# LLSean/ACE-Step-1.5-ggml

Measured on AMD Instinct MI355X. Metric: DiT denoising steps/sec (240s@5Hz latent, bs=1..8) + single-step ms; 1/2/4/8 GPU, higher is better.
Workload: dtype bf16

## Files before the change

ace-step-1.5-ggml_amd/csrc/kernels/gemm.hip:

```cpp
#include <array>
#include <cstdio>
#include <cstdlib>
#include <mutex>
#include <map>
#include <vector>
#include <type_traits>
#include <utility>

#include "gemm_common.h"

namespace acemi {
namespace gemm_detail {

#ifndef ACEMI_GEMM_ABLATE
#define ACEMI_GEMM_ABLATE 0
#endif
constexpr int kAblate = ACEMI_GEMM_ABLATE;


template <int TBM, int TBN, int TWM, int TWN, int TEPI, int TPIPE, bool TSK>
struct GemmTwoPerCU {
    static constexpr bool value =
        (TSK || ((TEPI == EPI_RESID || TEPI == EPI_RESID_GATED) && TPIPE >= 1 && TWM * TWN == 4 &&
                 (TBM / TWM / 16) * 4 * (TBN / TWN / 16) + (TEPI == EPI_RESID_GATED ? 2 * (TBN / TWN / 16) : 0) <= 63)) &&
// ... 193 lines not shown
            if (kt + 1 < nk) {
                if constexpr (PF)
                    wait_vmcnt<XW>();
                else
                    wait_retire(min(kt + NS, nk - 1) - (kt + 1));
                __builtin_amdgcn_s_barrier();
            }
        };
        if constexpr (XPF) {
            const int kp = nk >= 2 ? nk - 2 : 0;
            for (int kt = 0; kt < kp; ++kt) body(kt, std::false_type{});
            body(kp, std::true_type{});
            if (kp + 1 < nk) body(kp + 1, std::false_type{});
            resid_apply<TM, TN, EPI>(p, acc, m0 + wm0, n0 + wn0, lane, BM / WM, xo, g0, g1);
            return;
        } else {
            for (int kt = 0; kt < nk; ++kt) body(kt, std::false_type{});
        }
    }

    if constexpr (SK)
        if (!splitk_join<TM, TN, NW, SplitKMax<BM, BN>::value, NS * STAGE>(p, acc, S, sk_tile, sk_part, tid, smem,
                                                                                ticket0))
            return;
    if constexpr (EPI == EPI_QKV_PREP)
        qkv_prep_tile<BM, NW, TM, TN, NS * STAGE>(p, acc, m0, n0, wm0, wn0, tid, smem);
    else
        gemm_epilogue<TM, TN, F16, EPI, (SK ? 32 : (NW > 4 ? NW : 1024))>(p, acc, m0 + wm0, n0 + wn0, lane);
}


template <int BM, int BN, bool F16, int EPI, int NS>
__global__ void __launch_bounds__(512, 1) gemm_ws_kernel(GemmParams p) {
    constexpr int NC = 4, WN = 2;
    constexpr int WTM = BM / 2, WTN = BN / WN;
    constexpr int TM = WTM / 16, TN = WTN / 16;
    constexpr int BK = 64, ROWB = BK * 2;
    constexpr int STAGE = (BM + BN) * ROWB;
    constexpr int G = (BM + BN) / 8 / 4;
    static_assert((BM + BN) % 32 == 0 && NS >= 3, "ws tile");
    static_assert(EPI != EPI_SWIGLU || (TN % 2 == 0), "swiglu needs column pairs");
    __shared__ __attribute__((aligned(16))) char smem[NS * STAGE];

    const int tid = threadIdx.x, lane = tid & 63, wid = tid >> 6;
    int m0, n0;
    block_tile<BM, BN>(p, m0, n0);
    const int nk = p.K / BK;
    const uint32_t lds0 = (uint32_t)(uintptr_t)(__attribute__((address_space(3))) char*)smem;

    if (wid >= NC) {
        const int lw = wid - NC;
        const uint16_t* src[G];
#pragma unroll
        for (int j = 0; j < G; ++j) {
            const int row = (lw + 4 * j) * 8 + (lane >> 3);
            const int c = (lane & 7) ^ swz(row);
            src[j] = row < BM ? p.A + (int64_t)min(m0 + row, p.M - 1) * p.lda + c * 8
                              : p.W + (int64_t)(n0 + row - BM) * p.ldw + c * 8;
        }
        auto stage = [&](int slot, int kt) {
#pragma unroll
            for (int j = 0; j < G; ++j)
                __builtin_amdgcn_global_load_lds((const void*)(src[j] + kt * BK),
                                                 (lds_void*)(smem + slot * STAGE + (lw + 4 * j) * 1024), 16, 0, 0);
        };
        auto wait_tiles = [&](int n) {
            if (NS >= 4 && n >= 3) wait_vmcnt<(NS >= 4 ? 3 : 0) * G>();
            else if (n == 2) wait_vmcnt<2 * G>();
            else if (n == 1) wait_vmcnt<G>();
            else wait_vmcnt<0>();
        };
#pragma unroll
        for (int t = 0; t < NS; ++t)
            if (t < nk) stage(t, t);
        wait_tiles(min(NS, nk) - 1);
        __builtin_amdgcn_s_barrier();
        for (int j = 1; j < nk; ++j) {
            wait_tiles(min(nk - 1, j - 2 + NS) - j);
            __builtin_amdgcn_s_barrier();
            if (j - 1 + NS < nk) stage((j - 1) % NS, j - 1 + NS);
        }
        wait_vmcnt<0>();
        if constexpr (EPI == EPI_QKV_PREP)
            qkv_prep_head<BM, 8, NS * STAGE>(p, m0, n0 >> 7, tid, smem, [](float*, int, int) {});
        return;
    }

    const int wm0 = (wid / WN) * WTM, wn0 = (wid % WN) * WTN;
    const int lrow = lane & 15, lchunk = lane >> 4;
    const int rsw = (lrow >> 1) & 7;
    const uint32_t ch[2] = {(uint32_t)((lchunk ^ rsw) * 16), (uint32_t)(((4 + lchunk) ^ rsw) * 16)};
    f32x4 acc[TM][TN];
#pragma unroll
    for (int i = 0; i < TM; ++i)
#pragma unroll
        for (int j = 0; j < TN; ++j) acc[i][j] = f32x4{0.f, 0.f, 0.f, 0.f};
    uint4 a[TM][2], b[TN][2];
    auto rd = [&](auto r_c, int slot, auto h_c) {
        constexpr int r = decltype(r_c)::value, h = decltype(h_c)::value;
        const uint32_t sb = lds0 + slot * STAGE + ch[h];
        if constexpr (r < TN)
            b[r][h] = ds_read_b128_off<r * 16 * ROWB>(sb + (BM + wn0 + lrow) * ROWB);
        else
            a[r - TN][h] = ds_read_b128_off<(r - TN) * 16 * ROWB>(sb + (wm0 + lrow) * ROWB);
    };
    auto half = [&](auto h_c, int slot, auto hr_c, auto reads_c) {
        constexpr int h = decltype(h_c)::value;
        static_for<0, TM * TN>([&](auto s_c) {
            constexpr int st = decltype(s_c)::value;
            acc[st / TN][st % TN] = mfma16<F16>(a[st / TN][h], b[st % TN][h], acc[st / TN][st % TN]);
            if constexpr (decltype(reads_c)::value && st < TM + TN) rd(s_c, slot, hr_c);
            __builtin_amdgcn_sched_barrier(0);
        });
    };
    using H0 = std::integral_constant<int, 0>;
    using H1 = std::integral_constant<int, 1>;
    __builtin_amdgcn_s_barrier();
    static_for<0, TM + TN>([&](auto r_c) { rd(r_c, 0, H0{}); });
    lds_wait_all();
    using RD = std::true_type;
    for (int kt = 0; kt < nk - 1; ++kt) {
        half(H0{}, kt % NS, H1{}, RD{});
        lds_wait_all();
        __builtin_amdgcn_s_barrier();
        half(H1{}, (kt + 1) % NS, H0{}, RD{});
        lds_wait_all();
    }
    half(H0{}, (nk - 1) % NS, H1{}, RD{});
    lds_wait_all();
    half(H1{}, 0, H0{}, std::false_type{});
    if constexpr (EPI == EPI_QKV_PREP)
        qkv_prep_head<BM, 8, NS * STAGE>(p, m0, n0 >> 7, tid, smem, [&](float* tile, int c0, int CH) {
            const int ccol = lane & 15, crow = (lane >> 4) * 4;
#pragma unroll
            for (int i = 0; i < TM; ++i) {
                const int rb = wm0 + i * 16 - c0;
                if (rb < 0 || rb >= CH) continue;
#pragma unroll
                for (int r = 0; r < 4; ++r)
#pragma unroll
                    for (int j = 0; j < TN; ++j) tile[(rb + crow + r) * PREP_LD + wn0 + j * 16 + ccol] = acc[i][j][r];
            }
        });
    else
        gemm_epilogue<TM, TN, F16, EPI, 64>(p, acc, m0 + wm0, n0 + wn0, lane);
}

template <int BM, bool F16, int EPI, bool SK = false>
__global__ void __launch_bounds__(512) gemm8_kernel(GemmParams p) {
    constexpr int BN = 256, BK = 64, ROWB = BK * 2;
    constexpr int HA = BM / 2;
    constexpr int QM = BM / 64;
    constexpr int QN = 2;
    constexpr int PA = HA / 8;
    constexpr int STAGE = (BM + BN) * ROWB;
    constexpr int SCRATCH = 2 * STAGE;
    static_assert(BM == 256 || BM == 192, "gemm8 tile rows");
    static_assert(EPI != EPI_SWIGLU || (QN % 2 == 0), "swiglu needs column pairs");

    __shared__ __attribute__((aligned(16))) char smem[2 * STAGE + 16 * 1024];

    const int tid = threadIdx.x;
    const int lane = tid & 63;
    const int wid = tid >> 6;
    const int wr = wid >> 2, wc = wid & 3;
    int m0, n0, sk_tile = 0, sk_part = 0;
    unsigned ticket0 = 0;
    const int S = SK ? p.ksplit : 1;
    if constexpr (SK) {
        int ntiles;
        splitk_block(S, sk_tile, sk_part, ntiles);
        block_tile<BM, BN>(p, m0, n0, sk_tile, ntiles);
        if (tid == 0) ticket0 = __hip_atomic_fetch_add(p.sk_cnt + sk_tile, 1u, __ATOMIC_RELAXED, __HIP_MEMORY_SCOPE_AGENT);
    } else {
        block_tile<BM, BN>(p, m0, n0);
    }
    const int M = p.M;
    const int nk_all = p.K / BK;
    const int kt_begin = sk_part * nk_all / S;
    const int nk = (sk_part + 1) * nk_all / S - kt_begin;

    constexpr bool A2 = PA == 16;
    const bool a_second = A2 || wid + 8 < PA;
    const int prow = wid * 8 + (lane >> 3);
    const int pch = (lane & 7) ^ swz(prow);
    const uint16_t* srcA[2][2];
    const uint16_t* srcB[2][2];
#pragma unroll
    for (int h = 0; h < 2; ++h)
#pragma unroll
        for (int j = 0; j < 2; ++j) {
            const int ra = min(m0 + h * HA + j * 64 + prow, M - 1);
            srcA[h][j] = p.A + (int64_t)ra * p.lda + pch * 8 + kt_begin * BK;
            srcB[h][j] = p.W + (int64_t)(n0 + h * 128 + j * 64 + prow) * p.ldw + pch * 8 + kt_begin * BK;
        }
    auto stage_a = [&](int h, int t) {
        char* dst = t < nk ? smem + (t & 1) * STAGE + h * HA * ROWB : smem + SCRATCH;
        const int kt = min(t, nk - 1);
        __builtin_amdgcn_global_load_lds((const void*)(srcA[h][0] + kt * BK), (lds_void*)(dst + wid * 1024), 16, 0, 0);
        if (a_second)
            __builtin_amdgcn_global_load_lds((const void*)(srcA[h][1] + kt * BK), (lds_void*)(dst + (wid + 8) * 1024),
                                             16, 0, 0);
    };
    auto stage_b = [&](int h, int t) {
        char* dst = t < nk ? smem + (t & 1) * STAGE + (BM + h * 128) * ROWB : smem + SCRATCH;
        const int kt = min(t, nk - 1);
        __builtin_amdgcn_global_load_lds((const void*)(srcB[h][0] + kt * BK), (lds_void*)(dst + wid * 1024), 16, 0, 0);
        __builtin_amdgcn_global_load_lds((const void*)(srcB[h][1] + kt * BK), (lds_void*)(dst + (wid + 8) * 1024), 16,
                                         0, 0);
    };
    auto wait_stages = [&]() {
        if (a_second)
            wait_vmcnt<8>();
        else
            wait_vmcnt<6>();
    };

    const uint32_t lds0 = (uint32_t)(uintptr_t)(__attribute__((address_space(3))) char*)smem;
    const int lrow = lane & 15, lchunk = lane >> 4;
    const int rsw = (lrow >> 1) & 7;
    auto read_a = [&](int buf, int h, uint4 (&a)[QM][2]) {
        const uint32_t base = lds0 + buf * STAGE + (h * HA + wr * QM * 16 + lrow) * ROWB;
#pragma unroll
        for (int kk = 0; kk < 2; ++kk) ReadRows<0, QM, 16 * ROWB>::run(base + (((kk * 4 + lchunk) ^ rsw) * 16), a, kk);
// ... 3 lines not shown
#pragma unroll
        for (int kk = 0; kk < 2; ++kk) ReadRows<0, QN, 16 * ROWB>::run(base + (((kk * 4 + lchunk) ^ rsw) * 16), b, kk);
    };

    f32x4 acc[2][2][QM][QN];
#pragma unroll
    for (int x = 0; x < 2; ++x)
#pragma unroll
        for (int y = 0; y < 2; ++y)
#pragma unroll
            for (int i = 0; i < QM; ++i)
#pragma unroll
                for (int j = 0; j < QN; ++j) acc[x][y][i][j] = f32x4{0.f, 0.f, 0.f, 0.f};

    auto mma = [&](const uint4 (&a)[QM][2], const uint4 (&b)[QN][2], f32x4 (&c)[QM][QN]) {
        __builtin_amdgcn_s_setprio(1);
#pragma unroll
        for (int kk = 0; kk < 2; ++kk)
#pragma unroll
            for (int i = 0; i < QM; ++i)
#pragma unroll
                for (int j = 0; j < QN; ++j) c[i][j] = mfma16<F16>(a[i][kk], b[j][kk], c[i][j]);
        mfma_war_retire(a, b);
        __builtin_amdgcn_s_setprio(0);
    };
    auto seg = [&]() { __builtin_amdgcn_s_barrier(); };

    stage_a(0, 0);
    stage_b(0, 0);
    stage_b(1, 0);
    stage_a(1, 0);
    stage_a(0, 1);
    stage_b(0, 1);
    wait_stages();
    __builtin_amdgcn_s_barrier();
    if (wr == 1) __builtin_amdgcn_s_barrier();

    uint4 a[QM][2], b0[QN][2], b1[QN][2];
    for (int kt = 0; kt < nk; ++kt) {
        const int buf = kt & 1;
        if (!(kAblate & 2) || kt == 0) {
            read_a(buf, 0, a);
            read_b(buf, 0, b0);
        }
        if (!(kAblate & 1)) stage_b(1, kt + 1);
        wait_stages();
        seg();
        lds_wait_all();
        mma(a, b0, acc[0][0]);
        seg();
        if (!(kAblate & 2) || kt == 0) read_b(buf, 1, b1);
        if (!(kAblate & 1)) stage_a(1, kt + 1);
        wait_stages();
        seg();
        lds_wait_all();
        mma(a, b1, acc[0][1]);
        seg();
        if (!(kAblate & 2) || kt == 0) read_a(buf, 1, a);
        if (!(kAblate & 1)) stage_a(0, kt + 2);
        seg();
        lds_wait_all();
        mma(a, b1, acc[1][1]);
        seg();
        if (!(kAblate & 1)) stage_b(0, kt + 2);
        wait_stages();
        seg();
        __builtin_amdgcn_sched_barrier(0);
        mma(a, b0, acc[1][0]);
        seg();
    }
    if (wr == 0) __builtin_amdgcn_s_barrier();
    wait_vmcnt<0>();
    if constexpr (SK) {
        auto& acc2 = reinterpret_cast<f32x4 (&)[4 * QM][QN]>(acc);
        if (!splitk_join<4 * QM, QN, 8, SplitKMax<BM, BN>::value, 2 * STAGE + 16 * 1024>(p, acc2, S, sk_tile, sk_part, tid,
                                                                                        smem, ticket0))
            return;
    }

    if constexpr (EPI == EPI_QKV_PREP) {
        const int ccol = lane & 15, crow = (lane >> 4) * 4;
#pragma unroll
        for (int hb = 0; hb < 2; ++hb)
            qkv_prep_head<BM, 8, 2 * STAGE>(p, m0, (n0 >> 7) + hb, tid, smem, [&](float* tile, int c0, int CH) {
#pragma unroll
                for (int ha = 0; ha < 2; ++ha)
#pragma unroll
                    for (int i = 0; i < QM; ++i) {
                        const int rb = ha * HA + wr * QM * 16 + i * 16 - c0;
                        if (rb < 0 || rb >= CH) continue;
#pragma unroll
                        for (int r = 0; r < 4; ++r)
#pragma unroll
                            for (int j = 0; j < QN; ++j)
                                tile[(rb + crow + r) * PREP_LD + wc * 32 + j * 16 + ccol] = acc[ha][hb][i][j][r];
                    }
            });
    } else {
#pragma unroll
        for (int ha = 0; ha < 2; ++ha)
#pragma unroll
            for (int hb = 0; hb < 2; ++hb)
                gemm_epilogue<QM, QN, F16, EPI, 64>(p, acc[ha][hb], m0 + ha * HA + wr * QM * 16,
                                                   n0 + hb * 128 + wc * 32, lane);
    }
}

struct SplitKWs {
    void* ws = nullptr;
    size_t ws_bytes = 0;
    unsigned* cnt = nullptr;
    size_t tiles = 0;
};
std::mutex g_sk_mu;
std::map<std::pair<int, hipStream_t>, SplitKWs> g_sk;
std::map<int, unsigned*> g_sk_err;

unsigned* splitk_err_word(int dev) {
    unsigned*& e = g_sk_err[dev];
    if (!e) {
        ACEMI_HIP(hipHostMalloc(reinterpret_cast<void**>(&e), sizeof(unsigned), hipHostMallocMapped));
        *reinterpret_cast<volatile unsigned*>(e) = 0u;
    }
    return e;
}

void splitk_setup(GemmParams& p, int ntiles, int S, size_t tile_bytes, hipStream_t s) {
    int dev = 0;
    ACEMI_HIP(hipGetDevice(&dev));
    std::lock_guard<std::mutex> lk(g_sk_mu);
    SplitKWs& w = g_sk[std::make_pair(dev, s)];
    const size_t need = (size_t)ntiles * S * tile_bytes;
    if (w.ws_bytes < need || w.tiles < (size_t)ntiles) ACEMI_HIP(hipStreamSynchronize(s));
    if (w.ws_bytes < need) {
        if (w.ws) ACEMI_HIP(hipFree(w.ws));
        w.ws = nullptr;
        w.ws_bytes = 0;
        ACEMI_HIP(hipMalloc(&w.ws, need));
        w.ws_bytes = need;
    }
    if (w.tiles < (size_t)ntiles) {
        if (w.cnt) ACEMI_HIP(hipFree(w.cnt));
        w.cnt = nullptr;
        w.tiles = 0;
        const size_t t = std::max<size_t>((size_t)ntiles, 4096);
        ACEMI_HIP(hipMalloc(&w.cnt, 2 * t * sizeof(unsigned)));
        ACEMI_HIP(hipMemsetAsync(w.cnt, 0, 2 * t * sizeof(unsigned), s));
        w.tiles = t;
    }
    unsigned* err = splitk_err_word(dev);
    unsigned* err_dev = nullptr;
    ACEMI_HIP(hipHostGetDevicePointer(reinterpret_cast<void**>(&err_dev), err, 0));
    p.ksplit = S;
    p.sk_ws = static_cast<f32x4*>(w.ws);
    p.sk_cnt = w.cnt;
    p.sk_ready = w.cnt + w.tiles;
    p.sk_err = err_dev;
}

template <int BM, int BN, int WM, int WN, bool F16, int EPI, int PIPE, bool SK>
void launch_cfg(GemmParams p, int S, hipStream_t s) {
    static_assert(!SK || (WM * WN == 4 && PIPE >= 1), "split-K is for the 4-wave pipelined tiles");
    const int nbm = (p.M + BM - 1) / BM;
    const int nbn = p.N / BN;
    const dim3 grid(nbm * nbn * (S > 1 ? S : 1));
    const dim3 block(WM * WN * 64);
    if constexpr (EPI == EPI_QKV_PREP && BN != 128) {
        throw std::runtime_error("gemm: the fused attention prep needs 128-wide column tiles");
    } else {
        if constexpr (SK) {
            if (S > 1) {
                if (S > SplitKMax<BM, BN>::value) throw std::runtime_error("gemm: split-K factor too large for this tile");
                splitk_setup(p, nbm * nbn, S, (size_t)BM * BN * 4, s);
                hipLaunchKernelGGL((gemm_kernel<BM, BN, WM, WN, F16, EPI, PIPE, true>), grid, block, 0, s, p);
                return;
            }
        }
        hipLaunchKernelGGL((gemm_kernel<BM, BN, WM, WN, F16, EPI, PIPE>), grid, block, 0, s, p);
// ... 143 lines not shown
```

ace-step-1.5-ggml_amd/csrc/kernels/gemm_common.h:

```cpp
#pragma once

#include <algorithm>
#include <cmath>
#include <cstdlib>
#include <stdexcept>
#include <type_traits>

#include "../gemm_variants.h"
#include "../kernels.h"
#include "prep_math.h"
#include "mfma_guard.h"

namespace acemi {
namespace gemm_detail {

typedef __attribute__((ext_vector_type(8))) __bf16 bf16x8;
typedef __attribute__((ext_vector_type(8))) _Float16 f16x8;
typedef __attribute__((ext_vector_type(4))) float f32x4;

typedef __attribute__((address_space(3))) void lds_void;

struct GemmParams {
    const uint16_t* A;
    const uint16_t* W;
// ... 185 lines not shown
                        if (e.bias) v = v + bias_j[j];
                        e.c_act[(int64_t)m * e.ldc + n] = to_act<F16>(v);
                    } else if constexpr (EPI == EPI_PROJ_OUT) {
                        const int item = m / e.rows_per_item;
                        const int pp = m - item * e.rows_per_item;
                        const int kpos = n / e.out_ch;
                        const int c = n - kpos * e.out_ch;
                        const int t = pp * e.patch + kpos;
                        if (t < e.out_T) {
                            e.c_f32[((int64_t)item * e.out_T + t) * e.out_ch + c] = rn_add(v, e.bias[c]);
                        }
                    }
                }
            }
        }
    }
}

template <int TM, int TN, int EPI>
__device__ __forceinline__ void resid_prefetch(const GemmParams& p, int mw, int nw, int lane, int wrows,
                                               float (&xo)[TM][4][TN], float (&g0)[TN], float (&g1)[TN]) {
    const GemmEpilogue& e = p.e;
    const int ccol = lane & 15, crow = (lane >> 4) * 4;
#pragma unroll
    for (int i = 0; i < TM; ++i)
#pragma unroll
        for (int r = 0; r < 4; ++r) {
            const int m = min(mw + i * 16 + crow + r, p.M - 1);
#pragma unroll
            for (int j = 0; j < TN; ++j) xo[i][r][j] = e.c_f32[(int64_t)m * e.ldc + nw + j * 16 + ccol];
        }
    if constexpr (EPI == EPI_RESID_GATED) {
        const int i0 = min(mw, p.M - 1) / e.rows_per_item, i1 = min(mw + wrows - 1, p.M - 1) / e.rows_per_item;
#pragma unroll
        for (int j = 0; j < TN; ++j) {
            const int n = nw + j * 16 + ccol;
            g0[j] = e.gate[(int64_t)i0 * e.gate_stride + n];
            g1[j] = e.gate[(int64_t)i1 * e.gate_stride + n];
        }
    }
}

template <int TM, int TN, int EPI>
__device__ __forceinline__ void resid_apply(const GemmParams& p, f32x4 (&acc)[TM][TN], int mw, int nw, int lane,
                                            int wrows, const float (&xo)[TM][4][TN], const float (&g0)[TN],
                                            const float (&g1)[TN]) {
    const GemmEpilogue& e = p.e;
    const int ccol = lane & 15, crow = (lane >> 4) * 4;
    const int i0 = min(mw, p.M - 1) / e.rows_per_item;
    if (EPI != EPI_RESID_GATED || e.rows_per_item >= wrows) {
#pragma unroll
        for (int i = 0; i < TM; ++i)
#pragma unroll
            for (int r = 0; r < 4; ++r) {
                const int m = mw + i * 16 + crow + r;
                if (m >= p.M) continue;
                const bool first = m / e.rows_per_item == i0;
#pragma unroll
                for (int j = 0; j < TN; ++j) {
                    float v = acc[i][j][r];
                    if constexpr (EPI == EPI_RESID_GATED) v = rn_mul(v, first ? g0[j] : g1[j]);
                    e.c_f32[(int64_t)m * e.ldc + nw + j * 16 + ccol] = rn_add(xo[i][r][j], v);
                }
            }
    } else {
#pragma unroll
        for (int i = 0; i < TM; ++i)
#pragma unroll
            for (int r = 0; r < 4; ++r) {
                const int m = mw + i * 16 + crow + r;
                if (m >= p.M) continue;
                const int item = m / e.rows_per_item;
#pragma unroll
                for (int j = 0; j < TN; ++j) {
                    const int n = nw + j * 16 + ccol;
                    const float v = rn_mul(acc[i][j][r], e.gate[(int64_t)item * e.gate_stride + n]);
                    e.c_f32[(int64_t)m * e.ldc + n] = rn_add(xo[i][r][j], v);
                }
            }
    }
}

constexpr int PREP_LD = 144;

template <int BM, int NW, int SMEM, class Fill>
__device__ __forceinline__ void qkv_prep_head(const GemmParams& p, int m0, int hd, int tid, char* smem, Fill fill) {
    constexpr int LD = PREP_LD;
    constexpr int CH = (BM * LD * 4 <= SMEM) ? BM : ((BM / 2) * LD * 4 <= SMEM ? BM / 2 : BM / 4);
    static_assert(CH * LD * 4 <= SMEM && BM % CH == 0 && CH % 16 == 0, "qkv prep chunking");
    constexpr int NT = NW * 64;
    const PrepArgs& a = p.e.prep;
    float* tile = reinterpret_cast<float*>(smem);
    const int nq = a.q_col >= 0 ? a.hq : 0;
    const int nk = a.k_col >= 0 ? a.hkv : 0;
    for (int c0 = 0; c0 < BM; c0 += CH) {
        const int mc0 = m0 + c0;
        if (mc0 >= p.M) break;
        __syncthreads();
        fill(tile, c0, CH);
        __syncthreads();
        const int rows = min(CH, p.M - mc0);
        if (hd < nq + nk) {
            const bool isq = hd < nq;
            const int head = isq ? hd : hd - nq;
            const float* w = isq ? a.q_norm : a.k_norm;
            uint16_t* base = isq ? a.qh + (int64_t)head * a.n_pad * 128 : a.kh + (int64_t)head * a.n_pad * 128;
            const int64_t bstride = (int64_t)(isq ? a.hq : a.hkv) * a.n_pad * 128;
            const int64_t plane = isq ? a.q_plane : a.k_plane;
            const int d = (tid & 15) * 4;
            for (int t = tid >> 4; t < rows; t += NT / 16) {
                const int m = mc0 + t;
                const int b = m / a.n_tok, n = m - b * a.n_tok;
                const float4 x0 = *(const float4*)(tile + t * LD + d), x1 = *(const float4*)(tile + t * LD + 64 + d);
                float y[8] = {x0.x, x0.y, x0.z, x0.w, x1.x, x1.y, x1.z, x1.w};
                prep::head_row(y, w, d, a.eps, a.rope_cos ? a.rope_cos + (int64_t)n * 64 + d : nullptr,
                               a.rope_cos ? a.rope_sin + (int64_t)n * 64 + d : nullptr,
                               base + b * bstride + (int64_t)n * 128, plane, a.f8 ? (isq ? 1 : 2) : 0);
            }
        } else {
            const int hk = hd - nq - nk;
            const int d = tid & 127;
            const int b_lo = mc0 / a.n_tok, b_hi = (mc0 + rows - 1) / a.n_tok;
            for (int b = b_lo; b <= b_hi; ++b) {
                const int n_lo = max(0, mc0 - b * a.n_tok), n_hi = min(a.n_tok, mc0 + rows - b * a.n_tok);
                uint16_t* vdst = a.vt + (((int64_t)b * a.hkv + hk) * 128 + d) * a.n_pad;
                const int g_end = n_hi == a.n_tok ? a.n_pad / 16 : ((n_hi - 1) >> 4) + 1;
                for (int g = (n_lo >> 4) + (tid >> 7); g < g_end; g += NT / 128) {
                    const int g0 = g * 16;
                    float v[16];
                    uint32_t have = 0;
#pragma unroll
                    for (int k = 0; k < 16; ++k) {
                        const int n = g0 + prep::vperm(k);
                        const bool mine = n >= n_lo && n < n_hi;
                        v[k] = mine ? tile[(b * a.n_tok + n - mc0) * LD + d] : 0.f;
                        have |= (mine || n >= a.n_tok) ? (1u << k) : 0u;
                    }
                    uint32_t wv[8], wl[8];
                    prep::v_words(v, wv, wl);
                    if (a.f8 && a.v_plane > 0) {
                        float vn[16];
                        uint32_t hn = 0;
#pragma unroll
                        for (int w = 0; w < 16; ++w) {
                            vn[w] = v[prep::vperm(w)];
                            hn |= ((have >> prep::vperm(w)) & 1u) << w;
                        }
                        prep::v_store8(vn, vdst, a.v_plane, g0, hn);
                    }
                    if (have == 0xffffu) {
                        *(uint4*)(vdst + g0) = make_uint4(wv[0], wv[1], wv[2], wv[3]);
                        *(uint4*)(vdst + g0 + 8) = make_uint4(wv[4], wv[5], wv[6], wv[7]);
                        if (a.v_plane > 0 && !a.f8) {
                            *(uint4*)(vdst + a.v_plane + g0) = make_uint4(wl[0], wl[1], wl[2], wl[3]);
                            *(uint4*)(vdst + a.v_plane + g0 + 8) = make_uint4(wl[4], wl[5], wl[6], wl[7]);
                        }
                    } else {
#pragma unroll
                        for (int k = 0; k < 16; ++k) {
                            if (!((have >> k) & 1u)) continue;
                            vdst[g0 + k] = (uint16_t)(wv[k >> 1] >> (16 * (k & 1)));
                            if (a.v_plane > 0 && !a.f8) vdst[a.v_plane + g0 + k] = (uint16_t)(wl[k >> 1] >> (16 * (k & 1)));
                        }
                    }
                }
            }
        }
    }
}

template <int BM, int NW, int TM, int TN, int SMEM>
__device__ __forceinline__ void qkv_prep_tile(const GemmParams& p, f32x4 (&acc)[TM][TN], int m0, int n0, int wm0,
                                              int wn0, int tid, char* smem) {
    const int lane = tid & 63;
    const int ccol = lane & 15, crow = (lane >> 4) * 4;
    qkv_prep_head<BM, NW, SMEM>(p, m0, n0 >> 7, tid, smem, [&](float* tile, int c0, int CH) {
#pragma unroll
        for (int i = 0; i < TM; ++i) {
            const int rb = wm0 + i * 16 - c0;
            if (rb < 0 || rb >= CH) continue;
#pragma unroll
            for (int r = 0; r < 4; ++r)
#pragma unroll
                for (int j = 0; j < TN; ++j) tile[(rb + crow + r) * PREP_LD + wn0 + j * 16 + ccol] = acc[i][j][r];
        }
    });
}

constexpr int CPOL_SC1 = 16;

template <int BM, int BN>
struct SplitKMax {
    static constexpr int value = BM * BN >= 128 * 128 ? 2 : 4;
};

__device__ __forceinline__ void splitk_block(int S, int& tile, int& part, int& ntiles) {
    const int b = blockIdx.x;
    ntiles = gridDim.x / S;
    if ((ntiles & 7) == 0) {
        part = (b >> 3) % S;
        tile = (b / (8 * S)) * 8 + (b & 7);
    } else {
        part = b % S;
        tile = b / S;
    }
}

template <int TM, int TN, int NW, int SS, int SMEM>
__device__ __forceinline__ void splitk_gather(f32x4 (&acc)[TM][TN], const f32x4* slot0, int64_t slot_stride,
                                              int part, char* smem, int wid, int lane) {
    constexpr int F = TM * TN;
    constexpr int LDSW = SMEM / NW;
    constexpr int CH0 = LDSW / ((SS - 1) * 1024);
    constexpr int CH = CH0 < F ? CH0 : F;
    static_assert(CH >= 1, "split-K gather: LDS share too small");
    char* wl = smem + wid * LDSW;
#pragma unroll
    for (int f0 = 0; f0 < F; f0 += CH) {
        if (f0 > 0) lds_wait_all();
#pragma unroll
        for (int f = f0; f < f0 + CH && f < F; ++f)
#pragma unroll
            for (int qi = 0; qi < SS - 1; ++qi) {
                const int q = qi < part ? qi : qi + 1;
                __builtin_amdgcn_global_load_lds((const void*)(slot0 + q * slot_stride + f * 64),
                                                 (lds_void*)(wl + ((f - f0) * (SS - 1) + qi) * 1024), 16, 0,
                                                 CPOL_SC1);
            }
        wait_vmcnt<0>();
#pragma unroll
        for (int f = f0; f < f0 + CH && f < F; ++f) {
            if ((f - f0) % 4 == 0) __builtin_amdgcn_sched_barrier(0);
            const f32x4* l = reinterpret_cast<const f32x4*>(wl + (f - f0) * (SS - 1) * 1024) + lane;
            const int i = f / TN, j = f % TN;
            if constexpr (SS == 2) {
                acc[i][j] += l[0];
            } else {
                f32x4 t = part == 0 ? acc[i][j] : l[0];
#pragma unroll
                for (int q = 1; q < SS; ++q) t += q == part ? acc[i][j] : l[(q < part ? q : q - 1) * 64];
                acc[i][j] = t;
            }
        }
    }
}

template <int TM, int TN, int NW, int SKMAX, int SMEM>
__device__ __forceinline__ bool splitk_join(const GemmParams& p, f32x4 (&acc)[TM][TN], int S, int tile, int part,
                                           int tid, char* smem, unsigned ticket0) {
    __syncthreads();
    if (tid == 0) *reinterpret_cast<unsigned*>(smem) = ticket0;
    __syncthreads();
    const unsigned ticket = *reinterpret_cast<const unsigned*>(smem);
    __syncthreads();
    const bool last = ticket == (unsigned)(S - 1);
    const int wid = tid >> 6, lane = tid & 63;
    constexpr int PER_TILE = NW * TM * TN * 64;
    f32x4* slot0 = p.sk_ws + (int64_t)tile * S * PER_TILE + (wid * TM * TN) * 64 + lane;
    if (!last) {
        const __amdgpu_buffer_rsrc_t rs =
            __builtin_amdgcn_make_buffer_rsrc((void*)(slot0 - lane + (int64_t)part * PER_TILE), 0, 0x7fffffff, 0x00020000);
#pragma unroll
        for (int i = 0; i < TM; ++i)
#pragma unroll
            for (int j = 0; j < TN; ++j)
                __builtin_amdgcn_raw_buffer_store_b128(__builtin_bit_cast(u32x4, acc[i][j]), rs,
                                                       ((i * TN + j) * 64 + lane) * 16, 0, CPOL_SC1);
// ... 75 lines not shown
```

ace-step-1.5-ggml_amd/csrc/kernels/gemm_q.hip:

```cpp
#include "gemm_common.h"

namespace acemi {
namespace gemm_detail {

struct WRaw {
    u32x4 q0, q1;
    float s0, s1;
};

__device__ __forceinline__ uint32_t pk_bf16(float lo, float hi) {
    typedef __attribute__((ext_vector_type(2))) __bf16 bf16x2_t;
    bf16x2_t v;
    v[0] = (__bf16)lo;
    v[1] = (__bf16)hi;
    return __builtin_bit_cast(uint32_t, v);
}

__device__ __forceinline__ void ds_write_b128_v(uint32_t addr, uint32_t a, uint32_t b, uint32_t c, uint32_t d) {
    typedef __attribute__((address_space(3))) u32x4 lds_u32x4;
    *(lds_u32x4*)(uintptr_t)addr = u32x4{a, b, c, d};
}

template <int WQ>
__device__ __forceinline__ WRaw load_wq(const char* qbase, const float* sbase, int kt) {
// ... 400 lines not shown
#pragma unroll
        for (int j = 0; j < PA / NW; ++j)
            __builtin_amdgcn_global_load_lds((const void*)(srcA[j] + kt * BK), (lds_void*)(base + (wid + NW * j) * 1024),
                                             16, 0, 0);
#pragma unroll
        for (int j = 0; j < PQ / NW; ++j)
            __builtin_amdgcn_global_load_lds((const void*)(srcQ[j] + (int64_t)kt * QB),
                                             (lds_void*)(base + A_BYTES + (wid + NW * j) * 1024), 16, 0, 0);
#pragma unroll
        for (int j = 0; j < PS / NW; ++j)
            __builtin_amdgcn_global_load_lds((const void*)(srcS[j] + kt * (SB / 4)),
                                             (lds_void*)(base + A_BYTES + WQ_BYTES + (wid + NW * j) * 256), 4, 0, 0);
    };

    f32x4 acc[TM][TN];
#pragma unroll
    for (int i = 0; i < TM; ++i)
#pragma unroll
        for (int j = 0; j < TN; ++j) acc[i][j] = f32x4{0.f, 0.f, 0.f, 0.f};

    const uint32_t lds0 = (uint32_t)(uintptr_t)(__attribute__((address_space(3))) char*)smem;
    const int lrow = lane & 15, lchunk = lane >> 4;
    const int rsw = (lrow >> 1) & 7;

#pragma unroll
    for (int s = 0; s < RS - 1; ++s) stage(min(s, nk - 1), s);
    wait_vmcnt<G*(RS - 2)>();
    __builtin_amdgcn_s_barrier();
    for (int kt = 0; kt < nk; ++kt) {
        wait_vmcnt<G*(RS - 3)>();
        __builtin_amdgcn_s_barrier();
        stage(min(kt + RS - 1, nk - 1), (kt + RS - 1) % RS);
        const uint32_t sbase = lds0 + (kt % RS) * SLOT;
        const uint32_t abase = sbase + lrow * ROWB;
        QRaw raw;
        qd_read<WQ>(sbase + A_BYTES, sbase + A_BYTES + WQ_BYTES, wn0 + lrow, lchunk, raw);
        uint4 a0[TM][2], a1[TM][2], b[TN][2];
        ReadRows<0, TM, 16 * ROWB>::run(abase + (((0 * 4 + lchunk) ^ rsw) * 16), a0, 0);
        lds_wait_all();
        qd_dequant<WQ>(raw, lchunk, 0, b);
        mfma_war_guard();
        ReadRows<0, TM, 16 * ROWB>::run(abase + (((1 * 4 + lchunk) ^ rsw) * 16), a1, 1);
#pragma unroll
        for (int i = 0; i < TM; ++i)
#pragma unroll
            for (int j = 0; j < TN; ++j) acc[i][j] = mfma16<false>(a0[i][0], b[j][0], acc[i][j]);
        mfma_war_guard();
        qd_dequant<WQ>(raw, lchunk, 1, b);
        lds_wait_all();
        mfma_war_guard();
#pragma unroll
        for (int i = 0; i < TM; ++i)
#pragma unroll
            for (int j = 0; j < TN; ++j) acc[i][j] = mfma16<false>(a1[i][1], b[j][1], acc[i][j]);
        mfma_war_guard();
#ifdef ACEMI_QR_DIAG
        if constexpr (!SK) {
            QRaw raw2;
            qd_read<WQ>(sbase + A_BYTES, sbase + A_BYTES + WQ_BYTES, wn0 + lrow, lchunk, raw2);
            lds_wait_all();
            uint32_t* d = g_qr_dbg + ((size_t)(blockIdx.x * nk + kt) * (NW * 64) + tid) * 24;
            if ((size_t)(blockIdx.x * nk + kt + 1) * (NW * 64) * 24 <= (1u << 22)) {
#pragma unroll
                for (int j = 0; j < 2; ++j) {
                    d[j * 12 + 0] = raw.q[j][0][0]; d[j * 12 + 1] = raw.q[j][0][1];
                    d[j * 12 + 2] = raw.q[j][1][0]; d[j * 12 + 3] = raw.q[j][1][1];
                    d[j * 12 + 4] = raw.sc[j].x; d[j * 12 + 5] = raw.sc[j].y; d[j * 12 + 6] = raw.sc[j].z; d[j * 12 + 7] = raw.sc[j].w;
                    d[j * 12 + 8] = raw2.q[j][0][0]; d[j * 12 + 9] = raw2.q[j][1][0];
                    d[j * 12 + 10] = raw2.sc[j].x; d[j * 12 + 11] = raw2.sc[j].z;
                }
            }
        }
#endif
    }
    wait_vmcnt<0>();
    __syncthreads();

    if constexpr (SK)
        if (!splitk_join<TM, TN, NW, 4, RS * SLOT>(p, acc, S, sk_tile, sk_part, tid, smem, ticket0)) return;
    if constexpr (EPI == EPI_QKV_PREP) {
        const int ccol = lane & 15, crow = (lane >> 4) * 4;
#pragma unroll
        for (int hb = 0; hb < BN / 128; ++hb)
            qkv_prep_head<BM, NW, RS * SLOT>(p, m0, (n0 >> 7) + hb, tid, smem, [&](float* tile, int c0, int CH) {
                if ((wn0 >> 7) != hb) return;
#pragma unroll
                for (int i = 0; i < TM; ++i) {
                    const int rb = i * 16 - c0;
                    if (rb < 0 || rb >= CH) continue;
#pragma unroll
                    for (int r = 0; r < 4; ++r)
#pragma unroll
                        for (int j = 0; j < TN; ++j)
                            tile[(rb + crow + r) * PREP_LD + (wn0 & 127) + j * 16 + ccol] = acc[i][j][r];
                }
            });
    } else {
        gemm_epilogue<TM, TN, false, EPI, (SK ? 32 : 64)>(p, acc, m0, n0 + wn0, lane);
    }
}

template <int WQ>
__device__ __forceinline__ void wsq_read_raw(uint32_t q_addr, uint32_t s_addr, WRaw& r) {
    if constexpr (WQ == WF_Q4_K) {
        u32x4 q;
        uint2 sc;
        asm volatile("ds_read_b128 %0, %2\n\tds_read_b64 %1, %3\n\ts_waitcnt lgkmcnt(0)"
                     : "=&v"(q), "=&v"(sc) : "v"(q_addr), "v"(s_addr) : "memory");
        r.q0 = q;
        r.s0 = __uint_as_float(sc.x);
        r.s1 = __uint_as_float(sc.y);
    } else {
        u32x4 q0, q1;
        if constexpr (WQ == WF_Q8_0) {
            uint32_t sc;
            asm volatile("ds_read_b128 %0, %3\n\tds_read_b128 %1, %3 offset:16\n\tds_read_b32 %2, %4\n\ts_waitcnt lgkmcnt(0)"
                         : "=&v"(q0), "=&v"(q1), "=&v"(sc) : "v"(q_addr), "v"(s_addr) : "memory");
            r.s0 = __uint_as_float(sc);
            r.s1 = r.s0;
        } else {
            uint2 sc;
            asm volatile("ds_read_b128 %0, %3\n\tds_read_b128 %1, %3 offset:16\n\tds_read_b64 %2, %4\n\ts_waitcnt lgkmcnt(0)"
                         : "=&v"(q0), "=&v"(q1), "=&v"(sc) : "v"(q_addr), "v"(s_addr) : "memory");
            r.s0 = __uint_as_float(sc.x);
            r.s1 = __uint_as_float(sc.y);
        }
        r.q0 = q0;
        r.q1 = q1;
    }
}

template <int BM, int BN, int EPI, int WQ, int NS>
__global__ void __launch_bounds__(512, 1) gemm_wsq_kernel(GemmParams p) {
    constexpr int NC = 4, WN = 2;
    constexpr int WTM = BM / 2, WTN = BN / WN;
    constexpr int TM = WTM / 16, TN = WTN / 16;
    constexpr int BK = 64, ROWB = BK * 2;
    constexpr int STAGE = (BM + BN) * ROWB;
    constexpr int QB = QTile<WQ>::QB, SB = QTile<WQ>::SB;
    constexpr int RAW = BN * (QB + SB);
    constexpr int GA = BM / 8 / 4;
    constexpr int GQ = BN * QB / 1024 / 4;
    constexpr int GS = BN * SB / 256 / 4;
    constexpr int G = GA + GQ + GS;
    static_assert(BM % 32 == 0 && (BN * QB) % 4096 == 0 && (BN * SB) % 1024 == 0 && BN * 2 == 256, "wsq tile");
    static_assert(NS >= 3 && NS * (STAGE + RAW) <= 160 * 1024, "wsq ring");
    static_assert(EPI != EPI_SWIGLU || (TN % 2 == 0), "swiglu needs column pairs");
    __shared__ __attribute__((aligned(16))) char smem[NS * (STAGE + RAW)];

    const int tid = threadIdx.x, lane = tid & 63, wid = tid >> 6;
    int m0, n0;
    block_tile<BM, BN>(p, m0, n0);
    const int nk = p.K / BK;
    const uint32_t lds0 = (uint32_t)(uintptr_t)(__attribute__((address_space(3))) char*)smem;

    if (wid >= NC) {
        const int lw = wid - NC, ltid = tid - NC * 64;
        const uint16_t* srcA[GA];
#pragma unroll
        for (int j = 0; j < GA; ++j) {
            const int row = (lw + 4 * j) * 8 + (lane >> 3);
            const int c = (lane & 7) ^ swz(row);
            srcA[j] = p.A + (int64_t)min(m0 + row, p.M - 1) * p.lda + c * 8;
        }
        const int qrow_bytes = WQ == WF_Q4_K ? p.K / 2 : p.K;
        const int srow_floats = WQ == WF_Q8_0 ? p.K / 32 : p.K / 16;
        const char* srcQ[GQ];
#pragma unroll
        for (int j = 0; j < GQ; ++j) {
            constexpr int LPR = QB / 16;
            const int e = (lw * GQ + j) * 64 + lane;
            srcQ[j] = static_cast<const char*>(p.Wq) + (int64_t)(n0 + e / LPR) * qrow_bytes + (e % LPR) * 16;
        }
        const float* srcS[GS];
#pragma unroll
        for (int j = 0; j < GS; ++j) {
            constexpr int FPR = SB / 4;
            const int e = (lw * GS + j) * 64 + lane;
            srcS[j] = p.Ws + (int64_t)(n0 + e / FPR) * srow_floats + (e % FPR);
        }
        auto stage = [&](int t) {
            const int slot = t % NS;
            char* base = smem + slot * STAGE;
            char* raw = smem + NS * STAGE + slot * RAW;
#pragma unroll
            for (int j = 0; j < GQ; ++j)
                __builtin_amdgcn_global_load_lds((const void*)(srcQ[j] + (int64_t)t * QB),
                                                 (lds_void*)(raw + (lw * GQ + j) * 1024), 16, 0, 0);
#pragma unroll
            for (int j = 0; j < GS; ++j)
                __builtin_amdgcn_global_load_lds((const void*)(srcS[j] + t * (SB / 4)),
                                                 (lds_void*)(raw + BN * QB + (lw * GS + j) * 256), 4, 0, 0);
#pragma unroll
            for (int j = 0; j < GA; ++j)
                __builtin_amdgcn_global_load_lds((const void*)(srcA[j] + t * BK), (lds_void*)(base + (lw + 4 * j) * 1024), 16,
                                                 0, 0);
        };
        const int wr = ltid >> 1, wh = ltid & 1;
        const int wsw = swz(wr);
        constexpr int QOFF = WQ == WF_Q4_K ? 16 : 32;
        constexpr int SOFF = WQ == WF_Q8_0 ? 4 : 8;
        auto dequant = [&](int t, auto&& between) {
            const int slot = t % NS;
            const uint32_t raw = lds0 + NS * STAGE + slot * RAW;
            WRaw r;
            wsq_read_raw<WQ>(raw + wr * QB + wh * QOFF, raw + BN * QB + wr * SB + wh * SOFF, r);
            between();
            uint32_t o[16];
            dequant_block<WQ>(r, o);
            const uint32_t row = lds0 + slot * STAGE + (BM + wr) * ROWB;
            const uint32_t c0 = row + (((wh * 4 + 0) ^ wsw) * 16), c1 = row + (((wh * 4 + 1) ^ wsw) * 16);
            const uint32_t c2 = row + (((wh * 4 + 2) ^ wsw) * 16), c3 = row + (((wh * 4 + 3) ^ wsw) * 16);
            const u32x4 d0{o[0], o[1], o[2], o[3]}, d1{o[4], o[5], o[6], o[7]};
            const u32x4 d2{o[8], o[9], o[10], o[11]}, d3{o[12], o[13], o[14], o[15]};
            asm volatile(
                "ds_write_b128 %0, %4\n\tds_write_b128 %1, %5\n\tds_write_b128 %2, %6\n\tds_write_b128 %3, %7\n\t"
                "s_waitcnt lgkmcnt(0)"
                :
                : "v"(c0), "v"(c1), "v"(c2), "v"(c3), "v"(d0), "v"(d1), "v"(d2), "v"(d3)
                : "memory");
        };
        static_assert(NS == 3, "the counted waits below assume three ring slots");
#pragma unroll
        for (int t = 0; t < NS; ++t)
            if (t < nk) stage(t);
        if (nk > 2) wait_vmcnt<GA + G>();
        else if (nk == 2) wait_vmcnt<GA>();
        else wait_vmcnt<0>();
        __builtin_amdgcn_s_barrier();
        auto none = [] {};
        dequant(0, none);
        __builtin_amdgcn_s_barrier();
        for (int j = 1; j < nk; ++j) {
            dequant(j, none);
            if (j + 1 < nk) wait_vmcnt<GA>();
            else wait_vmcnt<0>();
            __builtin_amdgcn_s_barrier();
            if (j - 1 + NS < nk) stage(j - 1 + NS);
        }
        wait_vmcnt<0>();
        if constexpr (EPI == EPI_QKV_PREP)
            qkv_prep_head<BM, 8, NS * STAGE>(p, m0, n0 >> 7, tid, smem, [](float*, int, int) {});
        return;
    }

    const int wm0 = (wid / WN) * WTM, wn0 = (wid % WN) * WTN;
    const int lrow = lane & 15, lchunk = lane >> 4;
    const int rsw = (lrow >> 1) & 7;
    const uint32_t ch[2] = {(uint32_t)((lchunk ^ rsw) * 16), (uint32_t)(((4 + lchunk) ^ rsw) * 16)};
    f32x4 acc[TM][TN];
#pragma unroll
    for (int i = 0; i < TM; ++i)
#pragma unroll
        for (int j = 0; j < TN; ++j) acc[i][j] = f32x4{0.f, 0.f, 0.f, 0.f};
    uint4 a[TM][2], b[TN][2];
    auto rd = [&](auto r_c, int slot, auto h_c) {
        constexpr int r = decltype(r_c)::value, h = decltype(h_c)::value;
        const uint32_t sb = lds0 + slot * STAGE + ch[h];
        if constexpr (r < TN)
            b[r][h] = ds_read_b128_off<r * 16 * ROWB>(sb + (BM + wn0 + lrow) * ROWB);
        else
            a[r - TN][h] = ds_read_b128_off<(r - TN) * 16 * ROWB>(sb + (wm0 + lrow) * ROWB);
    };
    auto half = [&](auto h_c, int slot, auto hr_c, auto reads_c) {
        constexpr int h = decltype(h_c)::value;
        static_for<0, TM * TN>([&](auto s_c) {
            constexpr int st = decltype(s_c)::value;
            acc[st / TN][st % TN] = mfma16<false>(a[st / TN][h], b[st % TN][h], acc[st / TN][st % TN]);
            if constexpr (decltype(reads_c)::value && st < TM + TN) rd(s_c, slot, hr_c);
            __builtin_amdgcn_sched_barrier(0);
        });
    };
    using H0 = std::integral_constant<int, 0>;
    using H1 = std::integral_constant<int, 1>;
    __builtin_amdgcn_s_barrier();
    __builtin_amdgcn_s_barrier();
    static_for<0, TM + TN>([&](auto r_c) { rd(r_c, 0, H0{}); });
    lds_wait_all();
    using RD = std::true_type;
    for (int kt = 0; kt < nk - 1; ++kt) {
        half(H0{}, kt % NS, H1{}, RD{});
        lds_wait_all();
        __builtin_amdgcn_s_barrier();
        half(H1{}, (kt + 1) % NS, H0{}, RD{});
        lds_wait_all();
    }
    half(H0{}, (nk - 1) % NS, H1{}, RD{});
    lds_wait_all();
    half(H1{}, 0, H0{}, std::false_type{});
    mfma_war_guard();
    if constexpr (EPI == EPI_QKV_PREP)
        qkv_prep_head<BM, 8, NS * STAGE>(p, m0, n0 >> 7, tid, smem, [&](float* tile, int c0, int CH) {
            const int ccol = lane & 15, crow = (lane >> 4) * 4;
#pragma unroll
            for (int i = 0; i < TM; ++i) {
                const int rb = wm0 + i * 16 - c0;
                if (rb < 0 || rb >= CH) continue;
#pragma unroll
                for (int r = 0; r < 4; ++r)
#pragma unroll
                    for (int j = 0; j < TN; ++j) tile[(rb + crow + r) * PREP_LD + wn0 + j * 16 + ccol] = acc[i][j][r];
            }
        });
    else
        gemm_epilogue<TM, TN, false, EPI, 64>(p, acc, m0 + wm0, n0 + wn0, lane);
}

template <int BM, int BN, int EPI, int WQ, int NS>
void launch_wsq_cfg(const GemmParams& p, hipStream_t s) {
    if constexpr (EPI == EPI_QKV_PREP && BN != 128) {
        throw std::runtime_error("gemm: the fused attention prep needs 128-wide column tiles");
    } else {
        const int nbm = (p.M + BM - 1) / BM;
        hipLaunchKernelGGL((gemm_wsq_kernel<BM, BN, EPI, WQ, NS>), dim3(nbm * (p.N / BN)), dim3(512), 0, s, p);
    }
}

template <int BM, int BN, int WM, int WN, int EPI, int WQ>
void launch_q_cfg(const GemmParams& p, hipStream_t s) {
    const int nbm = (p.M + BM - 1) / BM;
    const int nbn = p.N / BN;
    if constexpr (EPI == EPI_QKV_PREP && BN != 128)
        throw std::runtime_error("gemm: the fused attention prep needs 128-wide column tiles");
    else
        hipLaunchKernelGGL((gemm_q_kernel<BM, BN, WM, WN, EPI, WQ>), dim3(nbm * nbn), dim3(WM * WN * 64), 0, s, p);
}

template <int BM, int NW, int EPI, int WQ, bool SK>
void launch_qr_cfg(GemmParams p, int S, hipStream_t s) {
    static_assert(!SK || (BM <= 128 && NW == 4), "split-K is for the 64 / 128-row quantized tiles");
    constexpr int BN = 32 * NW;
    const int nbm = (p.M + BM - 1) / BM;
    const int nbn = p.N / BN;
    if constexpr (SK) {
        if (S > 1) {
            splitk_setup(p, nbm * nbn, S, (size_t)BM * BN * 4, s);
            hipLaunchKernelGGL((gemm_qr_kernel<BM, NW, EPI, WQ, true>), dim3(nbm * nbn * S), dim3(NW * 64), 0, s, p);
            return;
        }
    }
    hipLaunchKernelGGL((gemm_qr_kernel<BM, NW, EPI, WQ>), dim3(nbm * nbn), dim3(NW * 64), 0, s, p);
}

template <int EPI, int WQ>
void launch_q_variant(int variant, const GemmParams& p, hipStream_t s) {
    const int S = check_variant_launch(variant, p.N, p.K, true);
    with_variant_row(variant % 100, [&](auto row) {
        constexpr GemmVariantRow r = GEMM_VARIANTS[decltype(row)::value];
        constexpr GemmKernelSel k = r.quant;
        if constexpr (k.family == GemmFamily::QTile) {
            static_assert(r.quant_split == 1, "split-K is for the register-dequant tiles");
            launch_q_cfg<k.bm, k.bn, k.wm, k.wn, EPI, WQ>(p, s);
        } else if constexpr (k.family == GemmFamily::QRing) {
            static_assert(r.quant_split <= 4, "the join gathers at most four parts");
            launch_qr_cfg<k.bm, k.wn, EPI, WQ, (r.quant_split > 1)>(p, S, s);
        } else if constexpr (k.family == GemmFamily::QWarpSpec) {
            static_assert(r.quant_split == 1, "no split-K for the warp-specialized quantized tile");
            launch_wsq_cfg<k.bm, k.bn, EPI, WQ, k.depth>(p, s);
        }
    });
}

template <int WQ>
void dispatch_q_epi(int variant, const GemmParams& p, hipStream_t s) {
    with_epilogue_kind(p.e.kind, [&](auto kind) { launch_q_variant<decltype(kind)::value, WQ>(variant, p, s); });
}

void dispatch_quant(int fmt, int variant, const GemmParams& p, hipStream_t s) {
    switch (fmt) {
        case WF_Q8_0: dispatch_q_epi<WF_Q8_0>(variant, p, s); break;
        case WF_Q4_K: dispatch_q_epi<WF_Q4_K>(variant, p, s); break;
        case WF_Q6_K: dispatch_q_epi<WF_Q6_K>(variant, p, s); break;
        default: throw std::runtime_error("gemm: bad quantized weight format");
    }
}

}

using namespace gemm_detail;

#ifdef ACEMI_QR_DIAG
extern "C" __attribute__((visibility("default"))) int ace_mi_qr_diag_read(uint32_t* out, size_t n_words, int clear) {
    if (n_words > (1u << 22)) return 2;
    if (out && hipMemcpyFromSymbol(out, HIP_SYMBOL(gemm_detail::g_qr_dbg), n_words * 4, 0, hipMemcpyDeviceToHost) != hipSuccess)
// ... 56 lines not shown
```

Measured before the change: 72.07.

## Write fused QKV-prep V transpose in full 64-key tiles with vector stores

Adds a tiled V-transpose path in the fused QKV-prep epilogue. Each full 64-key block is written with 16-byte stores per lane, covering the f16, lo-residual and fp8 planes, and the old per-16-group scalar path handles only the partial edges. The V staging tile uses a narrower row stride (130) to reduce LDS bank conflicts on the column reads. The chunk size now picks the largest multiple of 64 that fits in shared memory. The aim is to cut the cost of uncoalesced transposed V writes, at the price of more complex indexing and a risk of layout bugs.

```diff
diff --git a/ace-step-1.5-ggml_amd/csrc/kernels/gemm.hip b/ace-step-1.5-ggml_amd/csrc/kernels/gemm.hip
--- a/ace-step-1.5-ggml_amd/csrc/kernels/gemm.hip
+++ b/ace-step-1.5-ggml_amd/csrc/kernels/gemm.hip
@@ -299,7 +299,7 @@
         }
         wait_vmcnt<0>();
         if constexpr (EPI == EPI_QKV_PREP)
-            qkv_prep_head<BM, 8, NS * STAGE>(p, m0, n0 >> 7, tid, smem, [](float*, int, int) {});
+            qkv_prep_head<BM, 8, NS * STAGE>(p, m0, n0 >> 7, tid, smem, [](float*, int, int, int) {});
         return;
     }
 
@@ -347,7 +347,7 @@
     lds_wait_all();
     half(H1{}, 0, H0{}, std::false_type{});
     if constexpr (EPI == EPI_QKV_PREP)
-        qkv_prep_head<BM, 8, NS * STAGE>(p, m0, n0 >> 7, tid, smem, [&](float* tile, int c0, int CH) {
+        qkv_prep_head<BM, 8, NS * STAGE>(p, m0, n0 >> 7, tid, smem, [&](float* tile, int ld, int c0, int CH) {
             const int ccol = lane & 15, crow = (lane >> 4) * 4;
 #pragma unroll
             for (int i = 0; i < TM; ++i) {
@@ -356,7 +356,7 @@
 #pragma unroll
                 for (int r = 0; r < 4; ++r)
 #pragma unroll
-                    for (int j = 0; j < TN; ++j) tile[(rb + crow + r) * PREP_LD + wn0 + j * 16 + ccol] = acc[i][j][r];
+                    for (int j = 0; j < TN; ++j) tile[(rb + crow + r) * ld + wn0 + j * 16 + ccol] = acc[i][j][r];
             }
         });
     else
@@ -526,7 +526,7 @@
         const int ccol = lane & 15, crow = (lane >> 4) * 4;
 #pragma unroll
         for (int hb = 0; hb < 2; ++hb)
-            qkv_prep_head<BM, 8, 2 * STAGE>(p, m0, (n0 >> 7) + hb, tid, smem, [&](float* tile, int c0, int CH) {
+            qkv_prep_head<BM, 8, 2 * STAGE>(p, m0, (n0 >> 7) + hb, tid, smem, [&](float* tile, int ld, int c0, int CH) {
 #pragma unroll
                 for (int ha = 0; ha < 2; ++ha)
 #pragma unroll
@@ -537,7 +537,7 @@
                         for (int r = 0; r < 4; ++r)
 #pragma unroll
                             for (int j = 0; j < QN; ++j)
-                                tile[(rb + crow + r) * PREP_LD + wc * 32 + j * 16 + ccol] = acc[ha][hb][i][j][r];
+                                tile[(rb + crow + r) * ld + wc * 32 + j * 16 + ccol] = acc[ha][hb][i][j][r];
                     }
             });
     } else {
diff --git a/ace-step-1.5-ggml_amd/csrc/kernels/gemm_common.h b/ace-step-1.5-ggml_amd/csrc/kernels/gemm_common.h
--- a/ace-step-1.5-ggml_amd/csrc/kernels/gemm_common.h
+++ b/ace-step-1.5-ggml_amd/csrc/kernels/gemm_common.h
@@ -291,24 +291,74 @@
 }
 
 constexpr int PREP_LD = 144;
+constexpr int PREP_LD_V = 130;
+
+template <int NW>
+__device__ __forceinline__ void qkv_prep_vtile(const PrepArgs& a, const float* rows0, uint16_t* vhead, int key0,
+                                               int tid) {
+    constexpr int LD = PREP_LD_V;
+    const int lane = tid & 63, wid = tid >> 6;
+    const int e = lane & 1, h = (lane >> 1) & 1, c1 = lane >> 5;
+    const bool f8 = a.f8 && a.v_plane > 0;
+    for (int db = wid; db < 16; db += NW) {
+        const int d = db * 8 + ((lane >> 2) & 7);
+        const float* src = rows0 + (32 * c1 + 4 * h) * LD + d;
+        uint16_t* vrow = vhead + (int64_t)d * a.n_pad + key0;
+        float v[2][8];
+#pragma unroll
+        for (int i = 0; i < 2; ++i) {
+            if (!f8 && i != e) continue;
+#pragma unroll
+            for (int k = 0; k < 8; ++k) v[i][k] = src[(16 * i + 8 * (k >> 2) + (k & 3)) * LD];
+        }
+        float x[8];
+#pragma unroll
+        for (int k = 0; k < 8; ++k) x[k] = e ? v[1][k] : v[0][k];
+        uint32_t wv[4], wl[4];
+#pragma unroll
+        for (int j = 0; j < 4; ++j) {
+            const uint16_t h0 = prep::f16_bits(x[2 * j]), h1 = prep::f16_bits(x[2 * j + 1]);
+            wv[j] = (uint32_t)h0 | ((uint32_t)h1 << 16);
+            wl[j] = (uint32_t)prep::f16_bits(x[2 * j] - (float)__builtin_bit_cast(_Float16, h0)) |
+                    ((uint32_t)prep::f16_bits(x[2 * j + 1] - (float)__builtin_bit_cast(_Float16, h1)) << 16);
+        }
+        const int pos = 32 * c1 + 16 * e + 8 * h;
+        *(uint4*)(vrow + pos) = make_uint4(wv[0], wv[1], wv[2], wv[3]);
+        if (f8) {
+            uint32_t w8[4];
+#pragma unroll
+            for (int i = 0; i < 2; ++i)
+#pragma unroll
+                for (int q = 0; q < 2; ++q) {
+                    const float* y = &v[i][4 * q];
+                    w8[2 * i + q] = e ? prep::f8_pack4(y[0], y[1], y[2], y[3]) : prep::f8_lo_pack4(y[0], y[1], y[2], y[3]);
+                }
+            uint8_t* tile8 = reinterpret_cast<uint8_t*>(vhead + (int64_t)d * a.n_pad + a.v_plane) + 2 * key0;
+            *(uint4*)(tile8 + 64 * e + 16 * (c1 + 2 * h)) = make_uint4(w8[0], w8[1], w8[2], w8[3]);
+        } else if (a.v_plane > 0) {
+            *(uint4*)(vrow + a.v_plane + pos) = make_uint4(wl[0], wl[1], wl[2], wl[3]);
+        }
+    }
+}
 
 template <int BM, int NW, int SMEM, class Fill>
 __device__ __forceinline__ void qkv_prep_head(const GemmParams& p, int m0, int hd, int tid, char* smem, Fill fill) {
-    constexpr int LD = PREP_LD;
-    constexpr int CH = (BM * LD * 4 <= SMEM) ? BM : ((BM / 2) * LD * 4 <= SMEM ? BM / 2 : BM / 4);
-    static_assert(CH * LD * 4 <= SMEM && BM % CH == 0 && CH % 16 == 0, "qkv prep chunking");
+    constexpr int FIT = SMEM / (PREP_LD * 4);
+    constexpr int CH = BM <= FIT ? BM : (FIT >= 64 ? FIT / 64 * 64 : FIT / 16 * 16);
+    static_assert(CH >= 16 && CH * PREP_LD * 4 <= SMEM && PREP_LD_V <= PREP_LD, "qkv prep chunking");
     constexpr int NT = NW * 64;
     const PrepArgs& a = p.e.prep;
     float* tile = reinterpret_cast<float*>(smem);
     const int nq = a.q_col >= 0 ? a.hq : 0;
     const int nk = a.k_col >= 0 ? a.hkv : 0;
+    const int LD = hd < nq + nk ? PREP_LD : PREP_LD_V;
     for (int c0 = 0; c0 < BM; c0 += CH) {
         const int mc0 = m0 + c0;
         if (mc0 >= p.M) break;
         __syncthreads();
-        fill(tile, c0, CH);
+        fill(tile, LD, c0, CH);
         __syncthreads();
-        const int rows = min(CH, p.M - mc0);
+        const int rows = min(min(CH, BM - c0), p.M - mc0);
         if (hd < nq + nk) {
             const bool isq = hd < nq;
             const int head = isq ? hd : hd - nq;
@@ -332,9 +382,14 @@
             const int b_lo = mc0 / a.n_tok, b_hi = (mc0 + rows - 1) / a.n_tok;
             for (int b = b_lo; b <= b_hi; ++b) {
                 const int n_lo = max(0, mc0 - b * a.n_tok), n_hi = min(a.n_tok, mc0 + rows - b * a.n_tok);
-                uint16_t* vdst = a.vt + (((int64_t)b * a.hkv + hk) * 128 + d) * a.n_pad;
+                uint16_t* vhead = a.vt + ((int64_t)b * a.hkv + hk) * 128 * a.n_pad;
+                const int t_lo = (n_lo + 63) >> 6, t_hi = n_hi >> 6;
+                for (int t = t_lo; t < t_hi; ++t)
+                    qkv_prep_vtile<NW>(a, tile + (b * a.n_tok + t * 64 - mc0) * LD, vhead, t * 64, tid);
+                uint16_t* vdst = vhead + (int64_t)d * a.n_pad;
                 const int g_end = n_hi == a.n_tok ? a.n_pad / 16 : ((n_hi - 1) >> 4) + 1;
                 for (int g = (n_lo >> 4) + (tid >> 7); g < g_end; g += NT / 128) {
+                    if ((g >> 2) >= t_lo && (g >> 2) < t_hi) continue;
                     const int g0 = g * 16;
                     float v[16];
                     uint32_t have = 0;
@@ -383,7 +438,7 @@
                                               int wn0, int tid, char* smem) {
     const int lane = tid & 63;
     const int ccol = lane & 15, crow = (lane >> 4) * 4;
-    qkv_prep_head<BM, NW, SMEM>(p, m0, n0 >> 7, tid, smem, [&](float* tile, int c0, int CH) {
+    qkv_prep_head<BM, NW, SMEM>(p, m0, n0 >> 7, tid, smem, [&](float* tile, int ld, int c0, int CH) {
 #pragma unroll
         for (int i = 0; i < TM; ++i) {
             const int rb = wm0 + i * 16 - c0;
@@ -391,7 +446,7 @@
 #pragma unroll
             for (int r = 0; r < 4; ++r)
 #pragma unroll
-                for (int j = 0; j < TN; ++j) tile[(rb + crow + r) * PREP_LD + wn0 + j * 16 + ccol] = acc[i][j][r];
+                for (int j = 0; j < TN; ++j) tile[(rb + crow + r) * ld + wn0 + j * 16 + ccol] = acc[i][j][r];
         }
     });
 }
diff --git a/ace-step-1.5-ggml_amd/csrc/kernels/gemm_q.hip b/ace-step-1.5-ggml_amd/csrc/kernels/gemm_q.hip
--- a/ace-step-1.5-ggml_amd/csrc/kernels/gemm_q.hip
+++ b/ace-step-1.5-ggml_amd/csrc/kernels/gemm_q.hip
@@ -506,7 +506,7 @@
         const int ccol = lane & 15, crow = (lane >> 4) * 4;
 #pragma unroll
         for (int hb = 0; hb < BN / 128; ++hb)
-            qkv_prep_head<BM, NW, RS * SLOT>(p, m0, (n0 >> 7) + hb, tid, smem, [&](float* tile, int c0, int CH) {
+            qkv_prep_head<BM, NW, RS * SLOT>(p, m0, (n0 >> 7) + hb, tid, smem, [&](float* tile, int ld, int c0, int CH) {
                 if ((wn0 >> 7) != hb) return;
 #pragma unroll
                 for (int i = 0; i < TM; ++i) {
@@ -516,7 +516,7 @@
                     for (int r = 0; r < 4; ++r)
 #pragma unroll
                         for (int j = 0; j < TN; ++j)
-                            tile[(rb + crow + r) * PREP_LD + (wn0 & 127) + j * 16 + ccol] = acc[i][j][r];
+                            tile[(rb + crow + r) * ld + (wn0 & 127) + j * 16 + ccol] = acc[i][j][r];
                 }
             });
     } else {
@@ -664,7 +664,7 @@
         }
         wait_vmcnt<0>();
         if constexpr (EPI == EPI_QKV_PREP)
-            qkv_prep_head<BM, 8, NS * STAGE>(p, m0, n0 >> 7, tid, smem, [](float*, int, int) {});
+            qkv_prep_head<BM, 8, NS * STAGE>(p, m0, n0 >> 7, tid, smem, [](float*, int, int, int) {});
         return;
     }
 
@@ -714,7 +714,7 @@
     half(H1{}, 0, H0{}, std::false_type{});
     mfma_war_guard();
     if constexpr (EPI == EPI_QKV_PREP)
-        qkv_prep_head<BM, 8, NS * STAGE>(p, m0, n0 >> 7, tid, smem, [&](float* tile, int c0, int CH) {
+        qkv_prep_head<BM, 8, NS * STAGE>(p, m0, n0 >> 7, tid, smem, [&](float* tile, int ld, int c0, int CH) {
             const int ccol = lane & 15, crow = (lane >> 4) * 4;
 #pragma unroll
             for (int i = 0; i < TM; ++i) {
@@ -723,7 +723,7 @@
 #pragma unroll
                 for (int r = 0; r < 4; ++r)
 #pragma unroll
-                    for (int j = 0; j < TN; ++j) tile[(rb + crow + r) * PREP_LD + wn0 + j * 16 + ccol] = acc[i][j][r];
+                    for (int j = 0; j < TN; ++j) tile[(rb + crow + r) * ld + wn0 + j * 16 + ccol] = acc[i][j][r];
             }
         });
     else
```

Measured after the change: 72.44 (median of 6 runs). Within noise of the previous version (+0.5%).
